# weentiaan/Video-latent-diffusion-panoptic-segmentation

Hardware: NVIDIA B200
Metric: panoptic frames/sec (DDIM-50, 384x1248 KITTI) (higher is better)
Workload: dtype bf16

## Files before the change

### video_latent_diffusion_panoptic_segmentation_b200/csrc/gemm_tc.cu

```cuda
#include <stdlib.h>
#include <string.h>

#include "gemm_tc_kernel.cuh"

namespace ldm_gemm {
#define LDM_GEMM_DECLARE(NAME)                                                                                      \
  cudaError_t NAME(bool pair, int grid, int smem_bytes, cudaStream_t stream, const CUtensorMap& tmA1,               \
                   const CUtensorMap& tmA2, const CUtensorMap& tmB, const CUtensorMap& tmO, const CUtensorMap& tmR, \
                   const CUtensorMap& tmE, const GemmParams& p);
LDM_GEMM_DECLARE(launch_gemm_staged)
LDM_GEMM_DECLARE(launch_gemm_geglu)
LDM_GEMM_DECLARE(launch_gemm_qkv)
LDM_GEMM_DECLARE(launch_gemm_direct)
LDM_GEMM_DECLARE(launch_gemm_convt)
LDM_GEMM_DECLARE(launch_gemm_split)
LDM_GEMM_DECLARE(launch_gemm_geglu_ln)
LDM_GEMM_DECLARE(launch_gemm_qkv_ln)
}

namespace {

using namespace ldm;
using namespace ldm_gemm;

// ... 136 lines not shown
  const int rem = m_tile - b * tiles_per_img;
  const int ty = rem / p.tiles_x, tx = rem - ty * p.tiles_x;
  const int ly = r / p.bw, lx = r - ly * p.bw;
  const int y = ty * p.bh + ly, x = tx * p.bw + lx;
  const int n = n_tile * p.block_n + cb * 16 + vec * 8;
  if (r >= p.bw * p.bh || y >= p.H || x >= p.W || n >= p.N) return;
  const long long grow = ((long long)b * p.H + y) * p.W + x;
  float f[8];
#pragma unroll
  for (int j = 0; j < 8; ++j) f[j] = tile[r][vec * 8 + j];
  if (p.bias) {
    const float4 b0 = __ldg(reinterpret_cast<const float4*>(p.bias + n)), b1 = __ldg(reinterpret_cast<const float4*>(p.bias + n + 4));
    f[0] += b0.x; f[1] += b0.y; f[2] += b0.z; f[3] += b0.w; f[4] += b1.x; f[5] += b1.y; f[6] += b1.z; f[7] += b1.w;
  }
  if (p.rowbias) {
    const float* rb = p.rowbias + (long long)b * p.N + n;
    const float4 b0 = __ldg(reinterpret_cast<const float4*>(rb)), b1 = __ldg(reinterpret_cast<const float4*>(rb + 4));
    f[0] += b0.x; f[1] += b0.y; f[2] += b0.z; f[3] += b0.w; f[4] += b1.x; f[5] += b1.y; f[6] += b1.z; f[7] += b1.w;
  }
  if (p.residual) {
    const uint4 u = ld_nc_v4(p.residual + grow * p.N + n);
    const float2 a0 = unpack_bf16(u.x), a1 = unpack_bf16(u.y), a2 = unpack_bf16(u.z), a3 = unpack_bf16(u.w);
    f[0] += a0.x; f[1] += a0.y; f[2] += a1.x; f[3] += a1.y; f[4] += a2.x; f[5] += a2.y; f[6] += a3.x; f[7] += a3.y;
  }
  if (p.silu) {
#pragma unroll
    for (int j = 0; j < 8; ++j) f[j] = silu_f(f[j]);
  }
  store_bf16x8(p.out + grow * p.N + n, f);
}

int pair_override() { return ldm_host::diag_env("LDM_GEMM_PAIR", -1); }

}

extern "C" int ldm_gemm_bf16(const ldm_gemm_desc* d, ldm_stream_t stream) {
  using namespace ldm_host;
  LDM_REQUIRE(d != nullptr, LDM_ERR_BAD_ARG, "ldm_gemm_bf16: null descriptor");
  LDM_REQUIRE(d->a1 && d->w, LDM_ERR_BAD_ARG, "ldm_gemm_bf16: null a1/w");
  const bool up2 = d->up2 != 0;
  const int a_stride = d->a_stride > 1 ? d->a_stride : 1;
  LDM_REQUIRE(d->taps == 1 || d->taps == 9 || (d->taps == 4 && up2), LDM_ERR_BAD_ARG,
              "ldm_gemm_bf16: taps must be 1 or 9, or 4 with up2 (got %d)", d->taps);
  LDM_REQUIRE(!up2 || (d->taps == 4 && a_stride == 1), LDM_ERR_BAD_ARG, "ldm_gemm_bf16: up2 needs taps = 4 and a dense A");
  LDM_REQUIRE(a_stride == 1 || (a_stride == 2 && d->taps == 9 && (d->a_pad == 0 || d->a_pad == 1) && d->a_H > 0 && d->a_W > 0),
              LDM_ERR_BAD_ARG, "ldm_gemm_bf16: a_stride = 2 needs taps = 9, a_pad in {0, 1} and the input extents a_H, a_W");
  LDM_REQUIRE(d->B > 0 && d->H > 0 && d->W > 0 && d->N > 0 && d->c1 > 0, LDM_ERR_BAD_SHAPE,
              "ldm_gemm_bf16: non-positive extent B=%d H=%d W=%d N=%d c1=%d", d->B, d->H, d->W, d->N, d->c1);
  const int c2 = d->a2 ? d->c2 : 0;
  LDM_REQUIRE(d->c1 % 8 == 0 && c2 % 8 == 0, LDM_ERR_ALIGNMENT, "ldm_gemm_bf16: channels must be multiples of 8");
  if (d->taps != 1 || d->a2)
    LDM_REQUIRE(d->c1 % 64 == 0 && c2 % 64 == 0, LDM_ERR_BAD_SHAPE,
                "ldm_gemm_bf16: conv3x3 / concat sources need channels %% 64 == 0 (c1=%d c2=%d)", d->c1, c2);
  const int flags = d->flags;
  GemmParams p{};
  p.B = d->B;
  p.H = d->H;
  p.W = d->W;
  if (d->taps == 1 && !(flags & LDM_GEMM_CONVT_LN_SILU) && !d->rowbias) {
    p.W = d->B * d->H * d->W;
    p.H = 1;
    p.B = 1;
  }
  pick_box(p.H, p.W, d->taps, &p.bw, &p.bh);
  p.tiles_x = (p.W + p.bw - 1) / p.bw;
  p.tiles_y = (p.H + p.bh - 1) / p.bh;
  p.m_tiles = p.tiles_x * p.tiles_y * p.B;
  p.kblocks1 = (d->c1 + kBlockK - 1) / kBlockK;
  p.kblocks = p.kblocks1 + (c2 + kBlockK - 1) / kBlockK;
  const long kblocks_total = (long)d->taps * p.kblocks;
  double cost1 = 0.0, cost2 = 0.0;
  const bool split_ok = d->splitk_ws && d->splitk_ws_bytes > 0 && d->block_n <= 0 && !d->row_stats_out && !up2 &&
                        !(flags & (LDM_GEMM_OUT_F32 | LDM_GEMM_OUT_NCHW_F32 | LDM_GEMM_QKV_SPLIT |
                                   LDM_GEMM_CONVT_LN_SILU | LDM_GEMM_GEGLU)) &&
                        d->N >= 64 && d->N % 8 == 0 && staged_enabled() && splitk_enabled() &&
                        (reinterpret_cast<uintptr_t>(d->splitk_ws) & 15) == 0;
  const long ws_floats = split_ok ? (long)((d->splitk_ws_bytes - kSplitCounterBytes) / 4) : 0;
  int sp1 = 1, sp2 = 1;
  const int bn1 = pick_block_n(d->N, p.m_tiles, kblocks_total, num_sms(), false, d->taps, &cost1, split_ok ? 16 : 1,
                               ws_floats, &sp1);
  const int bn2 = pick_block_n(d->N, p.m_tiles, kblocks_total, num_sms(), true, d->taps, &cost2, split_ok ? 16 : 1,
                               ws_floats, &sp2);
  const bool pair_ok = p.m_tiles >= 2 && !(flags & LDM_GEMM_CONVT_LN_SILU) &&
                       (d->block_n <= 0 || (pair_override() == 1 && d->block_n >= 64 && d->block_n % 32 == 0));
  bool pair = pair_ok && cost2 < cost1 && kblocks_total >= 32;
  if (pair_override() >= 0) pair = pair_ok && pair_override() != 0;
  const bool qkv_tma_enabled = diag_env("LDM_GEMM_QKV_TMA", 1) != 0;
  bool qkv_tma = false;
  if ((flags & LDM_GEMM_QKV_SPLIT) && qkv_tma_enabled && d->block_n <= 0 && (!d->bias || d->ln_stats) && !d->rowbias &&
      d->head_dim > 0 &&
      160 % d->head_dim == 0 && (d->heads * d->head_dim) % 160 == 0 && p.H == 1 && p.bw == kBlockM && p.bh == 1 &&
      d->dpad == ((d->head_dim + 63) / 64) * 64 && d->seq >= kBlockM && kblocks_total <= 6) {
    qkv_tma = true;
    pair = false;
  }
  int block_n = d->block_n > 0 ? d->block_n : (qkv_tma ? 160 : (pair ? bn2 : bn1));
  int split_k = d->block_n > 0 || qkv_tma ? 1 : (pair ? sp2 : sp1);
  if ((flags & LDM_GEMM_GEGLU) && d->block_n <= 0 && block_n < 128) block_n = 128;
  int up2_cout = 0;
  if (up2) {
    LDM_REQUIRE(d->N % 4 == 0 && (d->N / 4) % 64 == 0 && d->out_H == 2 * d->H && d->out_W == 2 * d->W && !d->residual &&
                    !d->rowbias && !d->row_stats_out && !d->a2 &&
                    !(flags & ~(LDM_GEMM_SILU)),
                LDM_ERR_BAD_ARG, "ldm_gemm_bf16: up2 needs N = 4 * cout (cout %% 64 == 0), out_H = 2H, out_W = 2W, "
                "one source and the plain bf16 epilogue");
    up2_cout = d->N / 4;
    if (d->block_n <= 0) {
      int bn = block_n;
      while (bn > 64 && up2_cout % bn != 0) bn -= 32;
      block_n = bn;
    }
    LDM_REQUIRE(up2_cout % block_n == 0 && block_n >= 64, LDM_ERR_BAD_ARG, "ldm_gemm_bf16: up2 block_n=%d does not divide cout=%d",
                block_n, up2_cout);
  }
  LDM_REQUIRE(block_n % 32 == 0 && block_n >= 32 && block_n <= 256, LDM_ERR_BAD_ARG, "ldm_gemm_bf16: block_n=%d",
              block_n);
  if (flags & LDM_GEMM_GEGLU) LDM_REQUIRE(d->N % 32 == 0, LDM_ERR_BAD_SHAPE, "GEGLU needs N %% 32 == 0");
  if (flags & LDM_GEMM_QKV_SPLIT) {
    const int Cqkv = d->heads * d->head_dim;
    const int nparts = Cqkv > 0 ? d->N / Cqkv : 0;
    const int part0 = d->qkv_part0;
    LDM_REQUIRE(d->heads > 0 && d->head_dim % 8 == 0 && d->N == nparts * Cqkv && nparts >= 1 && part0 >= 0 &&
                    part0 + nparts <= 3 && d->seq > 0 && d->seq_pad % 8 == 0 && d->dpad % 64 == 0 &&
                    (long long)d->B * d->H * d->W % d->seq == 0,
                LDM_ERR_BAD_SHAPE, "ldm_gemm_bf16: bad QKV split geometry");
    LDM_REQUIRE((part0 > 0 || d->q) && (part0 > 1 || part0 + nparts < 2 || d->k) && (part0 + nparts < 3 || d->vt),
                LDM_ERR_BAD_ARG, "ldm_gemm_bf16: QKV split needs the q / k / vt buffers of the parts it writes");
  } else {
    LDM_REQUIRE(d->out != nullptr, LDM_ERR_BAD_ARG, "ldm_gemm_bf16: null out");
    LDM_REQUIRE(d->N % 8 == 0, LDM_ERR_ALIGNMENT, "ldm_gemm_bf16: N must be a multiple of 8 (got %d)", d->N);
  }
  if (flags & LDM_GEMM_CONVT_LN_SILU) {
    LDM_REQUIRE(d->taps == 1 && d->N == 4 * block_n && d->bias && d->ln_gamma && d->ln_beta, LDM_ERR_BAD_SHAPE,
                "ldm_gemm_bf16: CONVT_LN_SILU needs taps=1, N=4*block_n, bias, ln params");
  }

  p.block_n = block_n;
  p.n_tiles = (d->N + block_n - 1) / block_n;
  p.N = d->N;
  p.taps = d->taps;
  p.ktap = d->c1 + c2;
  p.stage_bytes = kABytes + (pair ? block_n / 2 : block_n) * kBlockK * 2;
  p.stages = (kSmemBudget - (1024 + 256)  - kEpiStageBytes) / p.stage_bytes;
  if (p.stages > kMaxStages) p.stages = kMaxStages;
  LDM_REQUIRE(p.stages >= 2, LDM_ERR_BAD_SHAPE, "ldm_gemm_bf16: not enough shared memory for 2 stages");
  const int n_out = (flags & LDM_GEMM_GEGLU) ? d->N / 2 : d->N;
  const bool staged = !(flags & (LDM_GEMM_OUT_F32 | LDM_GEMM_OUT_NCHW_F32 | LDM_GEMM_QKV_SPLIT | LDM_GEMM_CONVT_LN_SILU)) &&
                      n_out >= 64 && n_out % 8 == 0 && block_n >= ((flags & LDM_GEMM_GEGLU) ? 128 : 64) && staged_enabled();
  p.flags = flags | debug_flags() | (staged ? kStagedStore : 0) | (qkv_tma ? kQkvStaged : 0);
  if (!staged || block_n < 64) split_k = 1;
  p.split_k = split_k;
  if (split_k > 1) {
    const long m_alloc = pair ? 2 * ((p.m_tiles + 1) / 2) : p.m_tiles;
    p.ws = reinterpret_cast<float*>(d->splitk_ws);
    p.ws_slice_stride = (long long)m_alloc * p.n_tiles * block_n * kBlockM;
  }
  p.bias = d->bias;
  p.rowbias = d->rowbias;
  p.residual = reinterpret_cast<const __nv_bfloat16*>(d->residual);
  p.out = d->out;
  p.q = reinterpret_cast<__nv_bfloat16*>(d->q);
  p.k = reinterpret_cast<__nv_bfloat16*>(d->k);
  p.vt = reinterpret_cast<__nv_bfloat16*>(d->vt);
  p.ln_gamma = d->ln_gamma;
  p.ln_beta = d->ln_beta;
  p.ln_eps = d->ln_eps;
  p.heads = d->heads;
  p.head_dim = d->head_dim;
  p.dpad = d->dpad;
  p.seq = d->seq;
  p.seq_pad = d->seq_pad;
  p.vt_rows = d->vt_rows > 0 ? d->vt_rows : d->head_dim;
  p.qkv_part0 = d->qkv_part0;
  if (flags & LDM_GEMM_QKV_SPLIT) {
    auto magic = [](long long dv) { return (unsigned long long)(((1ULL << 40) + (unsigned long long)dv - 1) / (unsigned long long)dv); };
    p.magic_seq = magic(d->seq);
    p.magic_c = magic((long long)d->heads * d->head_dim);
    p.magic_d = magic(d->head_dim);
    LDM_REQUIRE((long long)d->B * d->H * d->W * d->seq < (1LL << 40) && (long long)d->N * d->heads * d->head_dim < (1LL << 40),
                LDM_ERR_BAD_SHAPE, "ldm_gemm_bf16: QKV split extents too large for the multiply-shift division");
  }
  if (d->row_stats_out)
    LDM_REQUIRE(staged && !(flags & LDM_GEMM_GEGLU), LDM_ERR_BAD_ARG,
                "ldm_gemm_bf16: row_stats_out needs the plain bf16 [rows, N] epilogue (N >= 64, N %% 8 == 0)");
  if (d->ln_stats) {
    LDM_REQUIRE((flags & (LDM_GEMM_GEGLU | LDM_GEMM_QKV_SPLIT)) && d->ln_colsum && d->taps == 1 && !d->a2 && !d->rowbias &&
                    d->ln_parts == (d->c1 + 31) / 32 && d->N % 8 == 0,
                LDM_ERR_BAD_ARG, "ldm_gemm_bf16: ln_stats needs a GEGLU / QKV_SPLIT pointwise GEMM, ln_colsum and "
                "ln_parts == ceil(c1 / 32) (got %d for c1 = %d)", d->ln_parts, d->c1);
    LDM_REQUIRE((flags & LDM_GEMM_QKV_SPLIT) || staged, LDM_ERR_BAD_SHAPE,
                "ldm_gemm_bf16: the folded GEGLU needs the staged epilogue (N >= 128, N %% 32 == 0)");
  }
  p.row_stats = reinterpret_cast<float*>(d->row_stats_out);
  p.ln_stats = reinterpret_cast<const float*>(d->ln_stats);
  p.ln_colsum = d->ln_colsum;
  p.ln_parts = d->ln_parts;
  p.rows_total = (long long)d->B * d->H * d->W;
  p.ln_invc = 1.0f / (float)d->c1;
  p.ln_fold_eps = d->ln_fold_eps;
  p.a_stride = a_stride;
  p.a_pad = a_stride == 2 ? d->a_pad : 1;
  p.up2_cout = up2_cout;
  p.up2_ntiles = up2 ? up2_cout / block_n : 0;
  if (up2) LDM_REQUIRE(staged && split_k == 1, LDM_ERR_BAD_SHAPE, "ldm_gemm_bf16: up2 needs the staged epilogue");
  p.n_store = d->n_store > 0 ? d->n_store : d->N;
  p.img_px = (long long)d->H * d->W;

  CUtensorMap tmA1, tmA2, tmB;
  const uint64_t aW = a_stride == 2 ? (uint64_t)d->a_W : (uint64_t)p.W, aH = a_stride == 2 ? (uint64_t)d->a_H : (uint64_t)p.H;
  const uint32_t a_es[4] = {1, (uint32_t)a_stride, (uint32_t)a_stride, 1};
  if (a_stride == 2) {
    const long long pad_total = d->a_pad == 1 ? 2 : 1;
    LDM_REQUIRE(((long long)aH + pad_total - 3) / 2 + 1 == d->H && ((long long)aW + pad_total - 3) / 2 + 1 == d->W,
                LDM_ERR_BAD_SHAPE, "ldm_gemm_bf16: stride-2 extents: input %llux%llu with a_pad=%d does not give %dx%d",
                (unsigned long long)aH, (unsigned long long)aW, d->a_pad, d->H, d->W);
  }
  {
    const uint64_t dims[4] = {(uint64_t)d->c1, aW, aH, (uint64_t)p.B};
    const uint64_t str[3] = {(uint64_t)d->c1 * 2, (uint64_t)d->c1 * 2 * aW, (uint64_t)d->c1 * 2 * aW * aH};
    const uint32_t box[4] = {kBlockK, (uint32_t)(p.bw * a_stride), (uint32_t)(p.bh * a_stride), 1};
    int rc = make_tmap(&tmA1, d->a1, 4, dims, str, box, 2, true, a_es);
    if (rc) return rc;
  }
  if (c2 > 0) {
    const uint64_t dims[4] = {(uint64_t)c2, aW, aH, (uint64_t)p.B};
    const uint64_t str[3] = {(uint64_t)c2 * 2, (uint64_t)c2 * 2 * aW, (uint64_t)c2 * 2 * aW * aH};
    const uint32_t box[4] = {kBlockK, (uint32_t)(p.bw * a_stride), (uint32_t)(p.bh * a_stride), 1};
    int rc = make_tmap(&tmA2, d->a2, 4, dims, str, box, 2, true, a_es);
    if (rc) return rc;
  } else {
    tmA2 = tmA1;
  }
  {
    const uint64_t ktot = (uint64_t)d->taps * p.ktap;
    const uint64_t dims[2] = {ktot, (uint64_t)d->N};
    const uint64_t str[1] = {ktot * 2};
    const uint32_t box[2] = {kBlockK, (uint32_t)(pair ? block_n / 2 : block_n)};
    int rc = make_tmap(&tmB, d->w, 2, dims, str, box, 2, true);
    if (rc) return rc;
  }

  CUtensorMap tmO = tmB;
  if (staged && up2) {
    const uint64_t dims[4] = {(uint64_t)up2_cout, (uint64_t)d->out_W, (uint64_t)d->out_H, (uint64_t)p.B};
    const uint64_t str[3] = {(uint64_t)up2_cout * 2, (uint64_t)up2_cout * 2 * d->out_W,
                             (uint64_t)up2_cout * 2 * d->out_W * d->out_H};
    const uint32_t box[4] = {64, (uint32_t)(2 * p.bw), (uint32_t)(2 * p.bh), 1};
    const uint32_t es[4] = {1, 2, 2, 1};
    int rc = make_tmap(&tmO, d->out, 4, dims, str, box, 2, true, es);
    if (rc) return rc;
  } else if (staged) {
    const uint64_t dims[4] = {(uint64_t)n_out, (uint64_t)p.W, (uint64_t)p.H, (uint64_t)p.B};
    const uint64_t str[3] = {(uint64_t)n_out * 2, (uint64_t)n_out * 2 * p.W, (uint64_t)n_out * 2 * p.W * p.H};
    const uint32_t box[4] = {64, (uint32_t)p.bw, (uint32_t)p.bh, 1};
    int rc = make_tmap(&tmO, d->out, 4, dims, str, box, 2, true);
    if (rc) return rc;
  }

  const bool plain_mode = !(flags & (LDM_GEMM_CONVT_LN_SILU | LDM_GEMM_GEGLU | LDM_GEMM_QKV_SPLIT));
  const bool res_mma = d->residual && d->identity && plain_mode && kblocks_total <= resmma_max_kblocks() && d->N % 8 == 0;
  p.res_kblocks = res_mma ? (block_n + kBlockK - 1) / kBlockK : 0;
  CUtensorMap tmE = tmB;
  if (res_mma) {
    const uint64_t dims[2] = {256, 256};
    const uint64_t str[1] = {512};
    const uint32_t box[2] = {kBlockK, (uint32_t)(pair ? block_n / 2 : block_n)};
    int rc = make_tmap(&tmE, d->identity, 2, dims, str, box, 2, true);
    if (rc) return rc;
  }
  CUtensorMap tmR = tmB;
  if (res_mma) {
    const uint64_t dims[4] = {(uint64_t)d->N, (uint64_t)p.W, (uint64_t)p.H, (uint64_t)p.B};
    const uint64_t str[3] = {(uint64_t)d->N * 2, (uint64_t)d->N * 2 * p.W, (uint64_t)d->N * 2 * p.W * p.H};
    const uint32_t box[4] = {64, (uint32_t)p.bw, (uint32_t)p.bh, 1};
    int rc = make_tmap(&tmR, d->residual, 4, dims, str, box, 2, true);
    if (rc) return rc;
  }

  if (qkv_tma) {
    const uint64_t nimg = (uint64_t)((long long)d->B * d->H * d->W / d->seq);
    const uint64_t dims[4] = {(uint64_t)d->dpad, (uint64_t)d->seq, (uint64_t)d->heads, nimg};
    const uint64_t str[3] = {(uint64_t)d->dpad * 2, (uint64_t)d->dpad * 2 * d->seq, (uint64_t)d->dpad * 2 * d->seq * d->heads};
    const uint32_t box[4] = {64, (uint32_t)kBlockM, 1, 1};
    if (d->q) {
      int rc = make_tmap(&tmO, d->q, 4, dims, str, box, 2, true);
      if (rc) return rc;
    }
    if (d->k) {
      int rc = make_tmap(&tmR, d->k, 4, dims, str, box, 2, true);
      if (rc) return rc;
    }
  }

  const int smem_bytes = p.stages * p.stage_bytes + kEpiStageBytes + 1024  + 256 ;
  int grid;
  if (pair) {
    const int units = ((p.m_tiles + 1) / 2) * p.n_tiles * split_k;
    int clusters = num_sms() / 2;
    if (clusters > units) clusters = units;
    grid = 2 * clusters;
  } else {
    const int num_tiles = p.m_tiles * p.n_tiles * split_k;
    grid = num_sms();
    if (grid > num_tiles) grid = num_tiles;
  }
  cudaError_t e;
  const cudaStream_t st = as_stream(stream);
  if (flags & LDM_GEMM_CONVT_LN_SILU)
// ... 46 lines not shown
```

### video_latent_diffusion_panoptic_segmentation_b200/csrc/gemm_tc_kernel.cuh

```cuda
#pragma once
#include "common.cuh"
#include "host_util.h"

namespace ldm_gemm {

using namespace ldm;

constexpr int kBlockM = 128;
constexpr int kBlockK = 64;
constexpr int kABytes = kBlockM * kBlockK * 2;
constexpr int kMaxStages = 8;
constexpr int kEpiWarps = 8;
constexpr int kThreads = 64 + 32 * kEpiWarps;
constexpr int kSmemBudget = 227 * 1024;
constexpr int kEpiStageBytes = 2 * 16384 + 1280;
constexpr int kStagedStore = 1 << 20;
constexpr int kQkvStaged = 1 << 21;
constexpr int kDbgNoTma = 1 << 29;
constexpr int kDbgNoMma = 1 << 30;
constexpr int kDbgNoFence = 1 << 27;
constexpr int kDbgKeepCommit = 1 << 26;
constexpr int kDbgNoWait = 1 << 28;

struct GemmParams {
  int tiles_x, tiles_y, B, bw, bh, W, H;
  int m_tiles, n_tiles, block_n;
  int N, taps, kblocks1, kblocks, ktap;
  int stages, stage_bytes;
  int res_kblocks;
  int flags;
  const float* bias;
  const float* rowbias;
  const __nv_bfloat16* residual;
  void* out;
  __nv_bfloat16* q;
  __nv_bfloat16* k;
  __nv_bfloat16* vt;
  const float* ln_gamma;
  const float* ln_beta;
  float ln_eps;
  int heads, head_dim, dpad, seq, seq_pad, vt_rows;
  int qkv_part0;
  unsigned long long magic_seq, magic_c, magic_d;
  int a_stride;
  int a_pad;
  int up2_ntiles;
  int up2_cout;
  int n_store;
  long long img_px;
  float* row_stats;
  const float* ln_stats;
  const float* ln_colsum;
  int ln_parts;
  long long rows_total;
  float ln_invc, ln_fold_eps;
  int split_k;
  float* ws;
  long long ws_slice_stride;
};

__device__ __forceinline__ void store_bf16x8(__nv_bfloat16* dst, const float* v) {
  uint4 u;
  u.x = pack_bf16(v[0], v[1]);
  u.y = pack_bf16(v[2], v[3]);
  u.z = pack_bf16(v[4], v[5]);
  u.w = pack_bf16(v[6], v[7]);
  *reinterpret_cast<uint4*>(dst) = u;
}

enum { kEpiStaged = 0, kEpiGeglu = 1, kEpiQkv = 2, kEpiDirect = 3, kEpiConvT = 4, kEpiSplit = 5, kEpiGegluLn = 6, kEpiQkvLn = 7 };
// ... 152 lines not shown
          const int slice = item % split;
          ksteps = (int)((long long)kmain * (slice + 1) / split) - (int)((long long)kmain * slice / split) +
                   (slice == split - 1 ? p.res_kblocks : 0);
        }
        mbar_wait(&tempty_bar[as], aphase ^ 1);
        tc_fence_after();
        const uint32_t d_tmem = tmem_base + (uint32_t)as * 256u;
        for (int ks = 0; ks < ksteps; ++ks) {
          if (!(p.flags & kDbgNoWait)) {
            mbar_wait(&full_bar[stage], phase);
            if (!(p.flags & kDbgNoFence)) tc_fence_after();
          }
          const uint32_t sa = smem_u32(smem + stage * p.stage_bytes);
          const uint64_t da = umma_desc_k_sw128(sa);
          const uint64_t db = umma_desc_k_sw128(sa + kABytes);
          if (elect_one()) {
#pragma unroll
            for (int k = 0; k < kBlockK / 16; ++k) {
              if (p.flags & kDbgNoMma) break;
              const uint32_t dt = d_tmem;
              if (kPair)
                umma_bf16_pair(dt, da + (uint64_t)(2 * k), db + (uint64_t)(2 * k), idesc, (ks | k) != 0);
              else
                umma_bf16(dt, da + (uint64_t)(2 * k), db + (uint64_t)(2 * k), idesc, (ks | k) != 0);
            }
            if ((p.flags & kDbgNoWait) && !(p.flags & kDbgKeepCommit)) {
            } else if (kPair) umma_commit_pair(&empty_bar[stage]); else umma_commit(&empty_bar[stage]);
          }
          __syncwarp();
          if (++stage == p.stages) {
            stage = 0;
            phase ^= 1;
          }
        }
        if (elect_one()) {
          if (kPair) umma_commit_pair(&tfull_bar[as]); else umma_commit(&tfull_bar[as]);
        }
        __syncwarp();
        if (++as == 2) {
          as = 0;
          aphase ^= 1;
        }
      }
    }
    __syncwarp();
  } else {
    const int quad = warp & 3;
    const int half = (warp - 2) >> 2;
    const int r = quad * 32 + lane;
    constexpr bool geglu = kEpi == kEpiGeglu;
    constexpr bool staged = kEpi == kEpiStaged || kEpi == kEpiGeglu;
    const bool plain = kEpi == kEpiStaged || (kEpi == kEpiDirect && !(p.flags & LDM_GEMM_GEGLU));
    const bool epi_leader = threadIdx.x == 64;
    int sb = 0;
    int as = 0;
    uint32_t aphase = 0;
    constexpr int kLnPre = 20;
    [[maybe_unused]] float2 ln_pre[kLnPre];
    [[maybe_unused]] auto ln_issue = [&](int item2) {
      const int tile2 = kSplit ? item2 / split : item2;
      const int n_tile2 = tile2 / m_units;
      const int m_unit2 = tile2 - n_tile2 * m_units;
      const int m_tile2 = kPair ? 2 * m_unit2 + (int)rank : m_unit2;
      const int b2 = m_tile2 / tiles_per_img;
      const int rem2 = m_tile2 - b2 * tiles_per_img;
      const int ty2 = rem2 / p.tiles_x;
      const int tx2 = rem2 - ty2 * p.tiles_x;
      const int ly2 = r / p.bw, lx2 = r - ly2 * p.bw;
      const int y2 = ty2 * p.bh + ly2, x2 = tx2 * p.bw + lx2;
      const bool valid2 = (m_tile2 < p.m_tiles) && (r < p.bw * p.bh) && (y2 < p.H) && (x2 < p.W);
      const float2* sp = reinterpret_cast<const float2*>(p.ln_stats) + (((long long)b2 * p.H + y2) * p.W + x2);
#pragma unroll
      for (int j = 0; j < kLnPre; ++j)
        ln_pre[j] = (valid2 && j < p.ln_parts) ? __ldg(sp + (long long)j * p.rows_total) : make_float2(0.f, 0.f);
    };
    if constexpr (kLn) {
      if (worker < num_items) ln_issue(worker);
    }
    for (int item = worker; item < num_items; item += num_workers) {
      const int tile = kSplit ? item / split : item;
      const int slice = kSplit ? item - tile * split : 0;
      const int n_tile = tile / m_units;
      const int m_unit = tile - n_tile * m_units;
      const int m_tile = kPair ? 2 * m_unit + (int)rank : m_unit;
      const int b = m_tile / tiles_per_img;
      const int rem = m_tile - b * tiles_per_img;
      const int ty = rem / p.tiles_x;
      const int tx = rem - ty * p.tiles_x;
      const int ly = r / p.bw, lx = r - ly * p.bw;
      const int y = ty * p.bh + ly, x = tx * p.bw + lx;
      const bool valid = (m_tile < p.m_tiles) && (r < p.bw * p.bh) && (y < p.H) && (x < p.W);
      const long long grow = ((long long)b * p.H + y) * p.W + x;
      const int n0 = n_tile * p.block_n;
      int qkv_bi = 0, qkv_s = 0;
      const bool qkv_vec = kEpi == kEpiQkv && (p.seq % 8 == 0) && p.bh == 1 && p.bw == kBlockM;
      if (kEpi == kEpiQkv) {
        qkv_bi = (int)(((unsigned long long)grow * p.magic_seq) >> 40);
        qkv_s = (int)(grow - (long long)qkv_bi * p.seq);
      }

      float ln_a = 1.f, ln_c = 0.f;
      constexpr bool ln_fold = kLn;
      if constexpr (ln_fold) {
        float su = 0.f, sq = 0.f;
#pragma unroll
        for (int j = 0; j < kLnPre; ++j) {
          su += ln_pre[j].x;
          sq += ln_pre[j].y;
        }
        if (valid) {
          const float2* sp = reinterpret_cast<const float2*>(p.ln_stats) + grow;
          for (int i = kLnPre; i < p.ln_parts; i += 10) {
            float2 t[10];
#pragma unroll
            for (int j = 0; j < 10; ++j)
              t[j] = i + j < p.ln_parts ? __ldg(sp + (long long)(i + j) * p.rows_total) : make_float2(0.f, 0.f);
#pragma unroll
            for (int j = 0; j < 10; ++j) {
              su += t[j].x;
              sq += t[j].y;
            }
          }
        }
        const float mean = su * p.ln_invc;
        ln_a = rsqrtf(fmaxf(fmaf(-mean, mean, sq * p.ln_invc), 0.f) + p.ln_fold_eps);
        ln_c = -mean * ln_a;
        if (item + num_workers < num_items) ln_issue(item + num_workers);
      }
      const bool ln_smem = kEpi == kEpiQkv && ln_fold && p.block_n <= 160;
      float* sLn = reinterpret_cast<float*>(epi_smem + 2 * 16384);
      if (ln_smem) {
        named_bar_sync(1, 32 * kEpiWarps);
        const int t = threadIdx.x - 64;
        if (t < p.block_n) {
          const int n = n0 + t;
          sLn[t] = (p.bias && n < p.N) ? __ldg(p.bias + n) : 0.f;
          sLn[160 + t] = n < p.N ? __ldg(p.ln_colsum + n) : 0.f;
        }
        named_bar_sync(1, 32 * kEpiWarps);
      }
      uint4 rs[4][4];
      const bool use_res = !kSplit && plain && p.residual != nullptr && valid && p.res_kblocks == 0;
      if (use_res) {
        const __nv_bfloat16* rrow = p.residual + grow * p.N + n0;
#pragma unroll
        for (int ci = 0; ci < 4; ++ci) {
          const int c = staged ? (ci * 64 < p.block_n ? min(ci * 64, p.block_n - 64) + half * 32 : p.block_n)
                               : (2 * ci + half) * 32;
#pragma unroll
          for (int g = 0; g < 4; ++g)
            if (c < p.block_n && n0 + c + g * 8 < p.N) rs[ci][g] = ld_nc_v4(rrow + c + g * 8);
        }
      }

      constexpr bool tile_bias = staged && !kSplit && !kLn;
      if constexpr (tile_bias) {
        float* sbias = reinterpret_cast<float*>(epi_smem + 2 * 16384);
        const int t = threadIdx.x - 64;
        if (t < p.block_n) {
          const int n = n0 + t;
          float bv = 0.f;
          if (n < p.N) {
            if (p.bias) bv = __ldg(p.bias + n);
            if (p.rowbias) bv += __ldg(p.rowbias + (long long)b * p.N + n);
          }
          sbias[t] = bv;
        }
      }
      mbar_wait(&tfull_bar[as], aphase);
      tc_fence_after();
      const uint32_t t_addr = tmem_base + ((uint32_t)(quad * 32) << 16) + (uint32_t)as * 256u;

      if constexpr (kSplit) {
        const long long tile_off = ((long long)m_tile * p.n_tiles + n_tile) * (long long)(p.block_n * kBlockM);
        float* wdst = p.ws + (long long)slice * p.ws_slice_stride + tile_off + r;
        for (int c = half * 32; c < p.block_n; c += 64) {
          uint32_t v[32];
          tmem_ld32(t_addr + c, v);
          tmem_ld_wait();
#pragma unroll
          for (int j = 0; j < 32; ++j) wdst[(c + j) * kBlockM] = __uint_as_float(v[j]);
        }
      }

      if constexpr (kSplit) {
      } else if constexpr (kEpi == kEpiConvT) {
        if (half == 0) {
        const int cout = p.block_n;
        float mean = 0.f;
        for (int c = 0; c < cout; c += 32) {
          uint32_t v[32];
          tmem_ld32(t_addr + c, v);
          tmem_ld_wait();
#pragma unroll
          for (int j = 0; j < 32; ++j) mean += __uint_as_float(v[j]) + __ldg(&p.bias[n0 + c + j]);
        }
        mean /= (float)cout;
        float var = 0.f;
        for (int c = 0; c < cout; c += 32) {
          uint32_t v[32];
          tmem_ld32(t_addr + c, v);
          tmem_ld_wait();
#pragma unroll
          for (int j = 0; j < 32; ++j) {
            const float d = __uint_as_float(v[j]) + __ldg(&p.bias[n0 + c + j]) - mean;
            var += d * d;
          }
        }
        const float rstd = 1.0f / sqrtf(var / (float)cout + p.ln_eps);
        const int sub = n_tile;
        const long long orow = ((long long)b * (2 * p.H) + (2 * y + (sub >> 1))) * (2 * p.W) + (2 * x + (sub & 1));
        __nv_bfloat16* dst = reinterpret_cast<__nv_bfloat16*>(p.out) + orow * cout;
        for (int c = 0; c < cout; c += 32) {
          uint32_t v[32];
          tmem_ld32(t_addr + c, v);
          tmem_ld_wait();
          if (valid) {
#pragma unroll
            for (int g = 0; g < 4; ++g) {
              float o[8];
#pragma unroll
              for (int j = 0; j < 8; ++j) {
                const int cc = c + g * 8 + j;
                const float xn = (__uint_as_float(v[g * 8 + j]) + __ldg(&p.bias[n0 + cc]) - mean) * rstd;
                o[j] = silu_f(__ldg(&p.ln_gamma[cc]) * xn + __ldg(&p.ln_beta[cc]));
              }
              store_bf16x8(dst + c + g * 8, o);
            }
          }
        }
        }
      } else if constexpr (staged) {
        const int acc_w = geglu ? 128 : 64;
#pragma unroll
        for (int ob = 0; ob < 4; ++ob) {
          if (ob * acc_w >= p.block_n) break;
          const int c0 = min(ob * acc_w, p.block_n - acc_w);
          uint8_t* sbuf = epi_smem + sb * 16384;
          float* sbias = reinterpret_cast<float*>(epi_smem + 2 * 16384);
          float* sgsum = sbias + 128;
          if (epi_leader) bulk_wait_read1();
          if constexpr (!tile_bias) {
            const int t = threadIdx.x - 64;
            if (t < acc_w) {
              const int n = n0 + c0 + t;
              float bv = 0.f;
              if (n < p.N) {
                if (p.bias) bv = __ldg(p.bias + n);
                if (p.rowbias) bv += __ldg(p.rowbias + (long long)b * p.N + n);
              }
              sbias[t] = bv;
              if (ln_fold) sgsum[t] = n < p.N ? __ldg(p.ln_colsum + n) : 0.f;
            }
          }
          named_bar_sync(1, 32 * kEpiWarps);
          uint8_t* rowp = sbuf + r * 128;
#pragma unroll
          for (int cq = 0; cq < 2; ++cq) {
            if (!geglu && cq == 1) break;
            const int cc = geglu ? half * 64 + cq * 32 : half * 32;
            const int c = c0 + cc;
            uint32_t v[32];
            tmem_ld32(t_addr + c, v);
            const int nc = n0 + c;
            float f[32];
            {
              const float4* bp = reinterpret_cast<const float4*>(sbias + (tile_bias ? c : cc));
              if (ln_fold) {
                tmem_ld_wait();
                const float4* gp = reinterpret_cast<const float4*>(sgsum + cc);
#pragma unroll
                for (int g = 0; g < 8; ++g) {
                  const float4 bv = bp[g], gv = gp[g];
                  f[g * 4] = fmaf(ln_a, __uint_as_float(v[g * 4]), fmaf(ln_c, gv.x, bv.x));
                  f[g * 4 + 1] = fmaf(ln_a, __uint_as_float(v[g * 4 + 1]), fmaf(ln_c, gv.y, bv.y));
                  f[g * 4 + 2] = fmaf(ln_a, __uint_as_float(v[g * 4 + 2]), fmaf(ln_c, gv.z, bv.z));
                  f[g * 4 + 3] = fmaf(ln_a, __uint_as_float(v[g * 4 + 3]), fmaf(ln_c, gv.w, bv.w));
                }
              } else {
                float4 bv[8];
#pragma unroll
                for (int g = 0; g < 8; ++g) bv[g] = bp[g];
                tmem_ld_wait();
#pragma unroll
                for (int g = 0; g < 8; ++g) {
                  f[g * 4] = __uint_as_float(v[g * 4]) + bv[g].x;
                  f[g * 4 + 1] = __uint_as_float(v[g * 4 + 1]) + bv[g].y;
                  f[g * 4 + 2] = __uint_as_float(v[g * 4 + 2]) + bv[g].z;
                  f[g * 4 + 3] = __uint_as_float(v[g * 4 + 3]) + bv[g].w;
                }
              }
            }
            if (geglu) {
              float o[16];
#pragma unroll
              for (int j = 0; j < 16; ++j) o[j] = f[j] * gelu_erf_fast(f[16 + j]);
#pragma unroll
              for (int g = 0; g < 2; ++g) {
                uint4 u;
                u.x = pack_bf16(o[g * 8 + 0], o[g * 8 + 1]); u.y = pack_bf16(o[g * 8 + 2], o[g * 8 + 3]);
                u.z = pack_bf16(o[g * 8 + 4], o[g * 8 + 5]); u.w = pack_bf16(o[g * 8 + 6], o[g * 8 + 7]);
                *reinterpret_cast<uint4*>(rowp + ((((cc >> 5) * 2 + g) ^ (r & 7)) << 4)) = u;
              }
            } else {
              if (use_res) {
#pragma unroll
                for (int g = 0; g < 4; ++g) {
                  if (nc + g * 8 >= p.N) break;
                  const uint4 u = rs[ob][g];
                  const float2 a0 = unpack_bf16(u.x), a1 = unpack_bf16(u.y), a2 = unpack_bf16(u.z), a3 = unpack_bf16(u.w);
                  f[g * 8 + 0] += a0.x; f[g * 8 + 1] += a0.y; f[g * 8 + 2] += a1.x; f[g * 8 + 3] += a1.y;
                  f[g * 8 + 4] += a2.x; f[g * 8 + 5] += a2.y; f[g * 8 + 6] += a3.x; f[g * 8 + 7] += a3.y;
                }
              }
              if (p.flags & LDM_GEMM_SILU) {
#pragma unroll
                for (int j = 0; j < 32; ++j) f[j] = silu_f(f[j]);
              }
              float st_s = 0.f, st_q = 0.f;
#pragma unroll
              for (int g = 0; g < 4; ++g) {
                uint4 u;
                u.x = pack_bf16(f[g * 8 + 0], f[g * 8 + 1]); u.y = pack_bf16(f[g * 8 + 2], f[g * 8 + 3]);
                u.z = pack_bf16(f[g * 8 + 4], f[g * 8 + 5]); u.w = pack_bf16(f[g * 8 + 6], f[g * 8 + 7]);
                *reinterpret_cast<uint4*>(rowp + (((half * 4 + g) ^ (r & 7)) << 4)) = u;
                if (kEpi == kEpiStaged && p.row_stats) {
                  const float2 a0 = unpack_bf16(u.x), a1 = unpack_bf16(u.y), a2 = unpack_bf16(u.z), a3 = unpack_bf16(u.w);
                  st_s += ((a0.x + a0.y) + (a1.x + a1.y)) + ((a2.x + a2.y) + (a3.x + a3.y));
                  st_q = fmaf(a0.x, a0.x, st_q); st_q = fmaf(a0.y, a0.y, st_q); st_q = fmaf(a1.x, a1.x, st_q);
                  st_q = fmaf(a1.y, a1.y, st_q); st_q = fmaf(a2.x, a2.x, st_q); st_q = fmaf(a2.y, a2.y, st_q);
                  st_q = fmaf(a3.x, a3.x, st_q); st_q = fmaf(a3.y, a3.y, st_q);
                }
              }
              if (kEpi == kEpiStaged && p.row_stats && valid && nc < p.N)
                *reinterpret_cast<float2*>(p.row_stats + ((long long)(nc >> 5) * p.rows_total + grow) * 2) =
                    make_float2(st_s, st_q);
            }
          }
          fence_proxy_async_smem();
          named_bar_sync(1, 32 * kEpiWarps);
          if (epi_leader) {
            if (p.up2_ntiles > 0) {
              const int cls = n_tile / p.up2_ntiles;
              tma_store_4d(&tmO, sbuf, n0 + c0 - cls * p.up2_cout, 2 * tx * p.bw + (cls & 1), 2 * ty * p.bh + (cls >> 1), b);
            } else {
              const int ncol = geglu ? (n0 + c0) / 2 : n0 + c0;
              tma_store_4d(&tmO, sbuf, ncol, tx * p.bw, ty * p.bh, b);
            }
            bulk_commit();
          }
          sb ^= 1;
        }
      } else {
        bool qkv_done = false;
        if constexpr (kEpi == kEpiQkv) {
          const int C = p.heads * p.head_dim;
          const int part_in = n0 / C;
          const int which_t = part_in + p.qkv_part0;
          const long long grow0 = (long long)m_tile * kBlockM;
          const int bi0 = (int)(((unsigned long long)grow0 * p.magic_seq) >> 40);
          const int s0 = (int)(grow0 - (long long)bi0 * p.seq);
          const int nimg = (int)(((long long)p.W * p.H * p.B) / p.seq);
          if ((p.flags & kQkvStaged) && which_t < 2 && (s0 + kBlockM <= p.seq || bi0 + 1 >= nimg)) {
            const int head0 = (n0 - part_in * C) / p.head_dim;
            const int heads_in_tile = p.block_n / p.head_dim;
            const int blocks_per_head = p.dpad >> 6;
            for (int hd = 0; hd < heads_in_tile; ++hd) {
              for (int kb = 0; kb < blocks_per_head; ++kb) {
                uint8_t* sbuf = epi_smem + sb * 16384;
                if (epi_leader) bulk_wait_read1();
                named_bar_sync(1, 32 * kEpiWarps);
                const int cbase = hd * p.head_dim + kb * 64 + half * 32;
                int ng = ((hd + 1) * p.head_dim - cbase) >> 3;
                ng = ng < 0 ? 0 : (ng > 4 ? 4 : ng);
                uint32_t v[32];
#pragma unroll
                for (int g = 0; g < 4; ++g)
                  if (g < ng) tmem_ld8(t_addr + cbase + g * 8, v + g * 8);
                tmem_ld_wait();
                if (ln_fold) {
#pragma unroll
                  for (int g = 0; g < 4; ++g)
                    if (g < ng) {
                      const int cl = cbase + g * 8;
                      float4 g0, g1, b0, b1;
                      if (ln_smem) {
                        b0 = *reinterpret_cast<const float4*>(sLn + cl);
                        b1 = *reinterpret_cast<const float4*>(sLn + cl + 4);
                        g0 = *reinterpret_cast<const float4*>(sLn + 160 + cl);
                        g1 = *reinterpret_cast<const float4*>(sLn + 160 + cl + 4);
                      } else {
                        const int n = n0 + cl;
                        g0 = __ldg(reinterpret_cast<const float4*>(p.ln_colsum + n));
                        g1 = __ldg(reinterpret_cast<const float4*>(p.ln_colsum + n + 4));
                        b0 = make_float4(0.f, 0.f, 0.f, 0.f), b1 = b0;
                        if (p.bias) {
                          b0 = __ldg(reinterpret_cast<const float4*>(p.bias + n));
                          b1 = __ldg(reinterpret_cast<const float4*>(p.bias + n + 4));
                        }
                      }
                      const float gv[8] = {g0.x, g0.y, g0.z, g0.w, g1.x, g1.y, g1.z, g1.w};
                      const float bv[8] = {b0.x, b0.y, b0.z, b0.w, b1.x, b1.y, b1.z, b1.w};
// ... 135 lines not shown
            continue;
          }
          if (use_res) {
#pragma unroll
            for (int g = 0; g < 4; ++g) {
              if (nc + g * 8 >= p.N) break;
              const uint4 u = rs[ci][g];
              const float2 a0 = unpack_bf16(u.x), a1 = unpack_bf16(u.y), a2 = unpack_bf16(u.z), a3 = unpack_bf16(u.w);
              f[g * 8 + 0] += a0.x; f[g * 8 + 1] += a0.y; f[g * 8 + 2] += a1.x; f[g * 8 + 3] += a1.y;
              f[g * 8 + 4] += a2.x; f[g * 8 + 5] += a2.y; f[g * 8 + 6] += a3.x; f[g * 8 + 7] += a3.y;
            }
          }
          if (p.flags & LDM_GEMM_SILU) {
#pragma unroll
            for (int j = 0; j < 32; ++j) f[j] = silu_f(f[j]);
          }
          if (p.flags & LDM_GEMM_OUT_NCHW_F32) {
            const long long bi = grow / p.img_px, pix = grow - bi * p.img_px;
            float* dst = reinterpret_cast<float*>(p.out) + (bi * p.n_store) * p.img_px + pix;
#pragma unroll
            for (int j = 0; j < 32; ++j)
              if (nc + j < p.n_store) dst[(long long)(nc + j) * p.img_px] = f[j];
            continue;
          }
          if (p.flags & LDM_GEMM_OUT_F32) {
            float* dst = reinterpret_cast<float*>(p.out) + grow * p.N + nc;
#pragma unroll
            for (int g = 0; g < 8; ++g) {
              if (nc + g * 4 >= p.N) break;
              *reinterpret_cast<float4*>(dst + g * 4) = make_float4(f[g * 4], f[g * 4 + 1], f[g * 4 + 2], f[g * 4 + 3]);
            }
          } else {
            __nv_bfloat16* dst = reinterpret_cast<__nv_bfloat16*>(p.out) + grow * p.N + nc;
#pragma unroll
            for (int g = 0; g < 4; ++g) {
              if (nc + g * 8 >= p.N) break;
              store_bf16x8(dst + g * 8, f + g * 8);
            }
          }
        }
      }
      tc_fence_before();
      __syncwarp();
      if (lane == 0) {
        if (kPair) mbar_arrive_cluster(&tempty_bar[as], 0); else mbar_arrive(&tempty_bar[as]);
      }
      if (++as == 2) {
        as = 0;
        aphase ^= 1;
      }
    }
  }

  if (threadIdx.x == 64) bulk_wait_all();
  tc_fence_before();
  if (kPair) cluster_sync_all(); else __syncthreads();
  if (warp == 1) {
    tc_fence_after();
    if (kPair) tmem_dealloc_pair(tmem_base, 512); else tmem_dealloc(tmem_base, 512);
  }
}

}
```

Before: 9.340.

## Issue per-warp TMA stores in staged GEMM epilogue instead of CTA-wide barrier

Adds a warp-store mode for the staged GEMM epilogue. Each epilogue warp stages its own 32-row by 64-column slice into a private shared-memory slot and issues its own TMA store with a 32x1 box, which removes the named barrier across all eight epilogue warps and the single-leader store. Bias values are precomputed into registers per warp, and each warp now handles whole output blocks instead of half-columns. The cost is more, smaller TMA stores, stricter eligibility (bw multiple of 32, no up2, no split-K, no ln stats), and a per-warp bulk wait at exit.

```diff
diff --git a/video_latent_diffusion_panoptic_segmentation_b200/csrc/gemm_tc.cu b/video_latent_diffusion_panoptic_segmentation_b200/csrc/gemm_tc.cu
--- a/video_latent_diffusion_panoptic_segmentation_b200/csrc/gemm_tc.cu
+++ b/video_latent_diffusion_panoptic_segmentation_b200/csrc/gemm_tc.cu
@@ -212,7 +212,8 @@
   if (d->taps != 1 || d->a2)
     LDM_REQUIRE(d->c1 % 64 == 0 && c2 % 64 == 0, LDM_ERR_BAD_SHAPE,
                 "ldm_gemm_bf16: conv3x3 / concat sources need channels %% 64 == 0 (c1=%d c2=%d)", d->c1, c2);
-  const int flags = d->flags;
+  const int flags = d->flags & ~kNoWarpStore;
+  const bool warp_store_ok = !(d->flags & kNoWarpStore);
   GemmParams p{};
   p.B = d->B;
   p.H = d->H;
@@ -307,8 +308,10 @@
   const int n_out = (flags & LDM_GEMM_GEGLU) ? d->N / 2 : d->N;
   const bool staged = !(flags & (LDM_GEMM_OUT_F32 | LDM_GEMM_OUT_NCHW_F32 | LDM_GEMM_QKV_SPLIT | LDM_GEMM_CONVT_LN_SILU)) &&
                       n_out >= 64 && n_out % 8 == 0 && block_n >= ((flags & LDM_GEMM_GEGLU) ? 128 : 64) && staged_enabled();
-  p.flags = flags | debug_flags() | (staged ? kStagedStore : 0) | (qkv_tma ? kQkvStaged : 0);
   if (!staged || block_n < 64) split_k = 1;
+  const bool warp_store = staged && warp_store_ok && !up2 && split_k == 1 && !d->ln_stats &&
+                          (p.bw % 32 == 0 || (p.bh == 1 && p.W <= p.bw));
+  p.flags = flags | debug_flags() | (staged ? kStagedStore : 0) | (qkv_tma ? kQkvStaged : 0) | (warp_store ? kWarpStore : 0);
   p.split_k = split_k;
   if (split_k > 1) {
     const long m_alloc = pair ? 2 * ((p.m_tiles + 1) / 2) : p.m_tiles;
@@ -412,8 +415,8 @@
   } else if (staged) {
     const uint64_t dims[4] = {(uint64_t)n_out, (uint64_t)p.W, (uint64_t)p.H, (uint64_t)p.B};
     const uint64_t str[3] = {(uint64_t)n_out * 2, (uint64_t)n_out * 2 * p.W, (uint64_t)n_out * 2 * p.W * p.H};
-    const uint32_t box[4] = {64, (uint32_t)p.bw, (uint32_t)p.bh, 1};
-    int rc = make_tmap(&tmO, d->out, 4, dims, str, box, 2, true);
+    const uint32_t box_cta[4] = {64, (uint32_t)p.bw, (uint32_t)p.bh, 1}, box_warp[4] = {64, 32, 1, 1};
+    int rc = make_tmap(&tmO, d->out, 4, dims, str, warp_store ? box_warp : box_cta, 2, true);
     if (rc) return rc;
   }
 
diff --git a/video_latent_diffusion_panoptic_segmentation_b200/csrc/gemm_tc_kernel.cuh b/video_latent_diffusion_panoptic_segmentation_b200/csrc/gemm_tc_kernel.cuh
--- a/video_latent_diffusion_panoptic_segmentation_b200/csrc/gemm_tc_kernel.cuh
+++ b/video_latent_diffusion_panoptic_segmentation_b200/csrc/gemm_tc_kernel.cuh
@@ -14,8 +14,11 @@
 constexpr int kThreads = 64 + 32 * kEpiWarps;
 constexpr int kSmemBudget = 227 * 1024;
 constexpr int kEpiStageBytes = 2 * 16384 + 1280;
+constexpr int kWarpSlotBytes = 2 * 16384 / kEpiWarps;
 constexpr int kStagedStore = 1 << 20;
 constexpr int kQkvStaged = 1 << 21;
+constexpr int kWarpStore = 1 << 22;
+constexpr int kNoWarpStore = 1 << 23;
 constexpr int kDbgNoTma = 1 << 29;
 constexpr int kDbgNoMma = 1 << 30;
 constexpr int kDbgNoFence = 1 << 27;
@@ -274,6 +277,9 @@
     constexpr bool staged = kEpi == kEpiStaged || kEpi == kEpiGeglu;
     const bool plain = kEpi == kEpiStaged || (kEpi == kEpiDirect && !(p.flags & LDM_GEMM_GEGLU));
     const bool epi_leader = threadIdx.x == 64;
+    const bool wstore = staged && !kLn && (p.flags & kWarpStore);
+    uint8_t* wslot = epi_smem + (warp - 2) * kWarpSlotBytes;
+    float* wbias_s = reinterpret_cast<float*>(epi_smem + 2 * 16384) + (warp - 2) * 32;
     int sb = 0;
     int as = 0;
     uint32_t aphase = 0;
@@ -367,7 +373,8 @@
         const __nv_bfloat16* rrow = p.residual + grow * p.N + n0;
 #pragma unroll
         for (int ci = 0; ci < 4; ++ci) {
-          const int c = staged ? (ci * 64 < p.block_n ? min(ci * 64, p.block_n - 64) + half * 32 : p.block_n)
+          const int obr = wstore ? half + 2 * (ci >> 1) : ci;
+          const int c = staged ? (obr * 64 < p.block_n ? min(obr * 64, p.block_n - 64) + (wstore ? (ci & 1) : half) * 32 : p.block_n)
                                : (2 * ci + half) * 32;
 #pragma unroll
           for (int g = 0; g < 4; ++g)
@@ -376,17 +383,29 @@
       }
 
       constexpr bool tile_bias = staged && !kSplit && !kLn;
+      constexpr int acc_w = geglu ? 128 : 64;
+      auto col_bias = [&](int t) {
+        const int n = n0 + t;
+        float bv = 0.f;
+        if (n < p.N) {
+          if (p.bias) bv = __ldg(p.bias + n);
+          if (p.rowbias) bv += __ldg(p.rowbias + (long long)b * p.N + n);
+        }
+        return bv;
+      };
+      constexpr int kChunks = acc_w / 32;
+      float wbias[2 * kChunks];
       if constexpr (tile_bias) {
-        float* sbias = reinterpret_cast<float*>(epi_smem + 2 * 16384);
-        const int t = threadIdx.x - 64;
-        if (t < p.block_n) {
-          const int n = n0 + t;
-          float bv = 0.f;
-          if (n < p.N) {
-            if (p.bias) bv = __ldg(p.bias + n);
-            if (p.rowbias) bv += __ldg(p.rowbias + (long long)b * p.N + n);
-          }
-          sbias[t] = bv;
+        if (wstore) {
+#pragma unroll
+          for (int i = 0; i < 2 * kChunks; ++i) {
+            const int ob = half + 2 * (i / kChunks), cq = i % kChunks;
+            wbias[i] = ob * acc_w < p.block_n ? col_bias(min(ob * acc_w, p.block_n - acc_w) + cq * 32 + lane) : 0.f;
+          }
+        } else {
+          float* sbias = reinterpret_cast<float*>(epi_smem + 2 * 16384);
+          const int t = threadIdx.x - 64;
+          if (t < p.block_n) sbias[t] = col_bias(t);
         }
       }
       mbar_wait(&tfull_bar[as], aphase);
@@ -453,34 +472,34 @@
         }
         }
       } else if constexpr (staged) {
-        const int acc_w = geglu ? 128 : 64;
+        auto stage16 = [&](uint8_t* sbuf, int j, const uint4& u) {
+          *reinterpret_cast<uint4*>(sbuf + (wstore ? lane : r) * 128 + ((j ^ (lane & 7)) << 4)) = u;
+        };
+        const int q0 = quad * 32;
+        const bool wq_ok = q0 < p.bw * p.bh;
 #pragma unroll
         for (int ob = 0; ob < 4; ++ob) {
           if (ob * acc_w >= p.block_n) break;
           const int c0 = min(ob * acc_w, p.block_n - acc_w);
-          uint8_t* sbuf = epi_smem + sb * 16384;
+          if (wstore && (ob & 1) != half) continue;
+          uint8_t* sbuf = wstore ? wslot : epi_smem + sb * 16384;
           float* sbias = reinterpret_cast<float*>(epi_smem + 2 * 16384);
           float* sgsum = sbias + 128;
-          if (epi_leader) bulk_wait_read1();
-          if constexpr (!tile_bias) {
-            const int t = threadIdx.x - 64;
-            if (t < acc_w) {
-              const int n = n0 + c0 + t;
-              float bv = 0.f;
-              if (n < p.N) {
-                if (p.bias) bv = __ldg(p.bias + n);
-                if (p.rowbias) bv += __ldg(p.rowbias + (long long)b * p.N + n);
-              }
-              sbias[t] = bv;
-              if (ln_fold) sgsum[t] = n < p.N ? __ldg(p.ln_colsum + n) : 0.f;
-            }
-          }
-          named_bar_sync(1, 32 * kEpiWarps);
-          uint8_t* rowp = sbuf + r * 128;
-#pragma unroll
-          for (int cq = 0; cq < 2; ++cq) {
-            if (!geglu && cq == 1) break;
-            const int cc = geglu ? half * 64 + cq * 32 : half * 32;
+          if (!wstore) {
+            if (epi_leader) bulk_wait_read1();
+            if constexpr (!tile_bias) {
+              const int t = threadIdx.x - 64;
+              if (t < acc_w) {
+                sbias[t] = col_bias(c0 + t);
+                if (ln_fold) sgsum[t] = n0 + c0 + t < p.N ? __ldg(p.ln_colsum + n0 + c0 + t) : 0.f;
+              }
+            }
+            named_bar_sync(1, 32 * kEpiWarps);
+          }
+#pragma unroll
+          for (int cq = 0; cq < kChunks; ++cq) {
+            if (!wstore && cq == kChunks / 2) break;
+            const int cc = wstore ? cq * 32 : (geglu ? half * 64 + cq * 32 : half * 32);
             const int c = c0 + cc;
             uint32_t v[32];
             tmem_ld32(t_addr + c, v);
@@ -488,6 +507,12 @@
             float f[32];
             {
               const float4* bp = reinterpret_cast<const float4*>(sbias + (tile_bias ? c : cc));
+              if (wstore) {
+                __syncwarp();
+                wbias_s[lane] = wbias[(ob >> 1) * kChunks + cq];
+                __syncwarp();
+                bp = reinterpret_cast<const float4*>(wbias_s);
+              }
               if (ln_fold) {
                 tmem_ld_wait();
                 const float4* gp = reinterpret_cast<const float4*>(sgsum + cc);
@@ -513,6 +538,10 @@
                 }
               }
             }
+            if (wstore && cq == 0) {
+              if (lane == 0) bulk_wait_read0();
+              __syncwarp();
+            }
             if (geglu) {
               float o[16];
 #pragma unroll
@@ -522,14 +551,14 @@
                 uint4 u;
                 u.x = pack_bf16(o[g * 8 + 0], o[g * 8 + 1]); u.y = pack_bf16(o[g * 8 + 2], o[g * 8 + 3]);
                 u.z = pack_bf16(o[g * 8 + 4], o[g * 8 + 5]); u.w = pack_bf16(o[g * 8 + 6], o[g * 8 + 7]);
-                *reinterpret_cast<uint4*>(rowp + ((((cc >> 5) * 2 + g) ^ (r & 7)) << 4)) = u;
+                stage16(sbuf, (cc >> 5) * 2 + g, u);
               }
             } else {
               if (use_res) {
 #pragma unroll
                 for (int g = 0; g < 4; ++g) {
                   if (nc + g * 8 >= p.N) break;
-                  const uint4 u = rs[ob][g];
+                  const uint4 u = wstore ? rs[(ob >> 1) * 2 + cq][g] : rs[ob][g];
                   const float2 a0 = unpack_bf16(u.x), a1 = unpack_bf16(u.y), a2 = unpack_bf16(u.z), a3 = unpack_bf16(u.w);
                   f[g * 8 + 0] += a0.x; f[g * 8 + 1] += a0.y; f[g * 8 + 2] += a1.x; f[g * 8 + 3] += a1.y;
                   f[g * 8 + 4] += a2.x; f[g * 8 + 5] += a2.y; f[g * 8 + 6] += a3.x; f[g * 8 + 7] += a3.y;
@@ -545,7 +574,7 @@
                 uint4 u;
                 u.x = pack_bf16(f[g * 8 + 0], f[g * 8 + 1]); u.y = pack_bf16(f[g * 8 + 2], f[g * 8 + 3]);
                 u.z = pack_bf16(f[g * 8 + 4], f[g * 8 + 5]); u.w = pack_bf16(f[g * 8 + 6], f[g * 8 + 7]);
-                *reinterpret_cast<uint4*>(rowp + (((half * 4 + g) ^ (r & 7)) << 4)) = u;
+                stage16(sbuf, (cc >> 5) * 4 + g, u);
                 if (kEpi == kEpiStaged && p.row_stats) {
                   const float2 a0 = unpack_bf16(u.x), a1 = unpack_bf16(u.y), a2 = unpack_bf16(u.z), a3 = unpack_bf16(u.w);
                   st_s += ((a0.x + a0.y) + (a1.x + a1.y)) + ((a2.x + a2.y) + (a3.x + a3.y));
@@ -560,16 +589,25 @@
             }
           }
           fence_proxy_async_smem();
-          named_bar_sync(1, 32 * kEpiWarps);
-          if (epi_leader) {
-            if (p.up2_ntiles > 0) {
-              const int cls = n_tile / p.up2_ntiles;
-              tma_store_4d(&tmO, sbuf, n0 + c0 - cls * p.up2_cout, 2 * tx * p.bw + (cls & 1), 2 * ty * p.bh + (cls >> 1), b);
-            } else {
+          if (wstore) {
+            __syncwarp();
+            if (lane == 0 && wq_ok) {
               const int ncol = geglu ? (n0 + c0) / 2 : n0 + c0;
-              tma_store_4d(&tmO, sbuf, ncol, tx * p.bw, ty * p.bh, b);
-            }
-            bulk_commit();
+              tma_store_4d(&tmO, sbuf, ncol, tx * p.bw + q0 % p.bw, ty * p.bh + q0 / p.bw, b);
+              bulk_commit();
+            }
+          } else {
+            named_bar_sync(1, 32 * kEpiWarps);
+            if (epi_leader) {
+              if (p.up2_ntiles > 0) {
+                const int cls = n_tile / p.up2_ntiles;
+                tma_store_4d(&tmO, sbuf, n0 + c0 - cls * p.up2_cout, 2 * tx * p.bw + (cls & 1), 2 * ty * p.bh + (cls >> 1), b);
+              } else {
+                const int ncol = geglu ? (n0 + c0) / 2 : n0 + c0;
+                tma_store_4d(&tmO, sbuf, ncol, tx * p.bw, ty * p.bh, b);
+              }
+              bulk_commit();
+            }
           }
           sb ^= 1;
         }
@@ -811,7 +849,7 @@
     }
   }
 
-  if (threadIdx.x == 64) bulk_wait_all();
+  if (warp >= 2 && lane == 0) bulk_wait_all();
   tc_fence_before();
   if (kPair) cluster_sync_all(); else __syncthreads();
   if (warp == 1) {
```

After: 9.083 (median of 6 runs). -2.7%, worse.
